# Adelaide-Autonomous-Racing-Kit/ac-mpc

Hardware: AMD Instinct MI355X
Metric: candidate-trajectories/sec (horizon=50) (higher is better)
Workload: dtype f32; 1 GPU; monza (synthetic circuit): 4096 candidates x horizon 50 per solve per GPU, 4096 solves (poses) batched per launch (256 distinct poses); mode S rollout + cost + argmin + winner record; horizon=50, mode=S, layout=U[P][n][2][N], parallelism=candidate-sharded x1, one all-reduce(MIN) of 4096 packed keys per step

## Files before the change

### ac-mpc_amd/acmpc_amd/_capi.py

```python
from __future__ import annotations

import ctypes as C
import os
import threading
from typing import Optional

import numpy as np

from . import _build

OK, EINVAL, EHIP, ENODEVICE, ECAPACITY, ESTATE = 0, -1, -2, -3, -4, -5
MODE_SPATIAL, MODE_TEMPORAL, MODE_DYNAMIC = 0, 1, 2
DYNAMICS_COUNT = 26
MAX_VEHICLES = 8
MAX_SUBSTEPS = 16
MAX_LOG_STEPS = 512
MAX_GRIP_HYPOTHESES = 65536
ENSEMBLE_MEAN, ENSEMBLE_MAX = 0, 1
ENSEMBLE_REDUCE = {"mean": ENSEMBLE_MEAN, "max": ENSEMBLE_MAX}
LAYOUT_CANDIDATE_MAJOR, LAYOUT_STEP_MAJOR = 0, 1
COEF_STRIDE = {MODE_SPATIAL: 12, MODE_TEMPORAL: 8, MODE_DYNAMIC: 8}
STATE_FLOATS = {MODE_SPATIAL: 3, MODE_TEMPORAL: 3, MODE_DYNAMIC: 6}
REC_COST, REC_VIOLATION, REC_NFEASIBLE, REC_OWNER, REC_HEADER = 0, 1, 2, 3, 4
ROUND_SINGLE, ROUND_PAIR, ROUND_QUAD, ROUND_TRIO = 0, 1, 2, 3
ROUND_FIELDS = ("kernel", "fused_finalize", "traced", "chained", "frames_in_lds", "frames_tabulated", "tick_accepted",
                "tick_frames")


ROLLOUT_KERNELS = (("step", None), ("tile", None), ("rows", "lds"), ("rows", "scalar"))


class EngineError(RuntimeError):

    def __init__(self, code: int, message: str):
        super().__init__("acmpc error %d: %s" % (code, message))
        self.code = code


class Params(C.Structure):
    _fields_ = [
        ("struct_size", C.c_uint32),
        ("mode", C.c_int32),
        ("device", C.c_int32),
        ("max_problems", C.c_int32),
        ("max_candidates", C.c_int32),
        ("max_steps", C.c_int32),
        ("nn_back", C.c_int32),
        ("nn_ahead", C.c_int32),
        ("centre_update", C.c_int32),
        ("lq_candidate", C.c_int32),
        ("step_cost", C.c_double * 3),
        ("r_term", C.c_double * 2),
        ("final_cost", C.c_double * 3),
        ("u_min", C.c_double * 2),
        ("u_max", C.c_double * 2),
        ("margin", C.c_double),
        ("wheelbase", C.c_double),
# ... 969 lines not shown
```

### ac-mpc_amd/csrc/acmpc_capi.hip

```cpp
#include <cstdio>
#include <cstdlib>
#include <algorithm>
#include <new>

#include "acmpc_ctx.h"
#include "acmpc_frames.h"
#include "acmpc_lq.h"

using namespace acmpc::capi;

namespace {

thread_local std::string g_create_error;

}

namespace acmpc {
namespace capi __attribute__((visibility("hidden"))) {

int fail(const acmpc_ctx* ctx, int code, const std::string& msg) {
  if (ctx != nullptr) {
    ctx->err = msg;
  } else {
    g_create_error = msg;
// ... 213 lines not shown
  c->touched_device = true;
  const acmpc_params& p = c->prm;
  const size_t cand = static_cast<size_t>(p.max_problems) * p.max_candidates;
  ACMPC_HIP(c, alloc_once(&c->d_centre, static_cast<size_t>(p.max_problems) * p.max_steps * 2 * sizeof(float)));
  ACMPC_HIP(c, alloc_once(&c->d_uref, static_cast<size_t>(p.max_problems) * p.max_steps * 2 * sizeof(float)));
  if (c->stream == nullptr) ACMPC_HIP(c, hipStreamCreateWithFlags(&c->stream, hipStreamNonBlocking));
  if (p.mode != ACMPC_MODE_DYNAMIC) {
    ACMPC_TRY(ensure_matrix(c));
  }
  const size_t state_floats = p.mode == ACMPC_MODE_DYNAMIC ? acmpc::kDynamicStateFloats : 3;
  ACMPC_HIP(c, alloc_once(&c->d_x0, static_cast<size_t>(p.max_problems) * state_floats * sizeof(float)));
  ACMPC_HIP(c, alloc_once(&c->d_costs, cand * sizeof(float)));
  ACMPC_HIP(c, alloc_once(&c->d_records,
                          static_cast<size_t>(p.max_problems) * acmpc_record_floats(p.max_steps) * sizeof(float)));
  ACMPC_HIP(c, alloc_once(&c->d_keys, static_cast<size_t>(p.max_problems) * sizeof(int64_t)));
  ACMPC_TRY(ensure_tail_buffers(c));
  ACMPC_HIP(c, host_alloc_once(&c->h_keys, static_cast<size_t>(p.max_problems) * sizeof(int64_t)));
  ACMPC_HIP(c, host_alloc_once(&c->h_io, (static_cast<size_t>(p.max_problems) * (state_floats + acmpc_record_floats(p.max_steps)) + 4) * sizeof(float)));
  if (p.lq_candidate != 0 && c->h_lq == nullptr) {
    const size_t lq_bytes = static_cast<size_t>(p.max_problems) * p.max_steps * 2 * sizeof(float);
    ACMPC_HIP(c, host_alloc_once(&c->h_lq, lq_bytes));
    std::memset(c->h_lq, 0, lq_bytes);
  }
  c->staging_ready = true;
  return ACMPC_OK;
}

static const char* const kOptionNames[] = {
    "ACMPC_SHAPE", "ACMPC_T_PACK", "ACMPC_NO_TILE", "ACMPC_TILE_ROWS", "ACMPC_TILE_TABLE", "ACMPC_NO_TRIO_ROUNDS",
    "ACMPC_NO_QUAD_ROUNDS", "ACMPC_NO_PAIR_ROUNDS", "ACMPC_SOLO_REGISTERS", "ACMPC_SOLO_SPLIT", "ACMPC_NO_VERIFIED_SEARCH",
    "ACMPC_NO_SOLO", "ACMPC_NO_FUSED_FINALIZE", "ACMPC_NO_TRACED_FINALIZE", "ACMPC_NO_CHAINED_ROUNDS", "ACMPC_NO_GRAPH",
    "ACMPC_NO_FUSED_SAMPLING", "ACMPC_TICK_GRAPH", "ACMPC_TICK_NO_FLAG", "ACMPC_TICK_NO_INLINE_PATH", "ACMPC_NO_ZERO_COPY", "ACMPC_TAILED_ROLLOUT", "ACMPC_NO_GROUP_FINALIZE", "ACMPC_FINALIZE_WAVES",
    "ACMPC_NO_CHAINED_STREAM", "ACMPC_LQ_BOX_ITERATIONS", "ACMPC_START_CLOCKS", "ACMPC_DYNAMIC_MATRIX_ROUNDS",
    "ACMPC_CONFORMANT_SYNC"};

static bool apply_option(acmpc_ctx* c, const char* name, const char* value) {
  const std::string key(name);
  const bool present = value != nullptr && value[0] != '\0';
  const bool on = present && !(value[0] == '0' && value[1] == '\0');
  auto tri = [&](int* field) { *field = present ? (value[0] == '1' ? 1 : 0) : -1; return true; };
  acmpc::LaunchOptions& o = c->opt;
  if (key == "ACMPC_SHAPE") {
    o.shape_block = o.shape_cpt = 0;
    if (present && std::sscanf(value, "%d,%d", &o.shape_block, &o.shape_cpt) != 2) o.shape_block = o.shape_cpt = 0;
    return true;
  }
  if (key == "ACMPC_T_PACK") { o.temporal_pack = present ? (value[0] == '1' ? 1 : 2) : 0; return true; }
  if (key == "ACMPC_NO_TILE") { o.no_tile = on; return true; }
  if (key == "ACMPC_TILE_ROWS") { o.tile_rows = present ? std::atoi(value) : -1; return true; }
  if (key == "ACMPC_TILE_TABLE") { o.tile_table = present ? (value[0] == 'l' ? 1 : 2) : 0; return true; }
  if (key == "ACMPC_NO_TRIO_ROUNDS") { o.no_trio_rounds = on; return true; }
  if (key == "ACMPC_NO_QUAD_ROUNDS") { o.no_quad_rounds = on; return true; }
  if (key == "ACMPC_NO_PAIR_ROUNDS") { o.no_pair_rounds = on; return true; }
  if (key == "ACMPC_SOLO_REGISTERS") return tri(&o.solo_registers);
  if (key == "ACMPC_SOLO_SPLIT") return tri(&o.solo_split);
  if (key == "ACMPC_NO_GROUP_FINALIZE") { o.no_group_finalize = on; return true; }
  if (key == "ACMPC_FINALIZE_WAVES") { o.finalize_waves = on; return true; }
  acmpc_ctx::Switches& w = c->sw;
  if (key == "ACMPC_NO_VERIFIED_SEARCH") { w.no_verified_search = on; return true; }
  if (key == "ACMPC_NO_SOLO") { w.no_solo = on; return true; }
  if (key == "ACMPC_NO_FUSED_FINALIZE") { w.no_fused_finalize = on; return true; }
  if (key == "ACMPC_NO_TRACED_FINALIZE") { w.no_traced_finalize = on; return true; }
  if (key == "ACMPC_NO_CHAINED_ROUNDS") { w.no_chained_rounds = on; return true; }
  if (key == "ACMPC_NO_CHAINED_STREAM") { w.no_chained_stream = on; return true; }
  if (key == "ACMPC_NO_GRAPH") { w.no_graph = on; return true; }
  if (key == "ACMPC_NO_FUSED_SAMPLING") { w.no_fused_sampling = on; return true; }
  if (key == "ACMPC_TICK_GRAPH") { w.tick_graph = on; return true; }
  if (key == "ACMPC_TICK_NO_FLAG") { w.tick_no_flag = on; return true; }
  if (key == "ACMPC_TICK_NO_INLINE_PATH") { w.tick_no_inline_path = on; return true; }
  if (key == "ACMPC_NO_ZERO_COPY") { w.no_zero_copy = on; return true; }
  if (key == "ACMPC_TAILED_ROLLOUT") { w.tailed_rollout = on; return true; }
  if (key == "ACMPC_START_CLOCKS") { c->want_start_clocks = on; return true; }
  if (key == "ACMPC_DYNAMIC_MATRIX_ROUNDS") { w.dynamic_matrix_rounds = on; return true; }
  if (key == "ACMPC_CONFORMANT_SYNC") {
    w.no_solo = w.no_fused_finalize = w.no_chained_stream = w.tick_no_flag = on;
    if (on) w.tailed_rollout = false;
    return true;
  }
  if (key == "ACMPC_LQ_BOX_ITERATIONS") { c->lq_box_iterations = present ? std::max(0, std::atoi(value)) : 40; return true; }
  return false;
}

}
}

extern "C" {
// ... 319 lines not shown
```

### ac-mpc_amd/csrc/acmpc_capi_optimize.hip

```cpp
#include <algorithm>

#include "acmpc_ctx.h"
#include "acmpc_lq.h"

using namespace acmpc::capi;

namespace acmpc {
namespace capi __attribute__((visibility("hidden"))) {

static const float* own_frames(const acmpc_ctx* c) { return c->h_nn_frames.empty() ? nullptr : c->d_nn_frames; }

bool use_fused_finalize(const acmpc_ctx* c, int n) {
  return !c->sw.no_fused_finalize && acmpc::fused_finalize_fits(c->prm.mode, n);
}

RoundPlan plan_rounds(const acmpc_ctx* c, int P, int N, int n) {
  const int blocks = (N + 63) / 64;
  RoundPlan plan{};
  plan.fused_finalize = use_fused_finalize(c, n);
  plan.traced = plan.fused_finalize && !c->sw.no_traced_finalize && acmpc::traced_finalize_fits(c->prm.mode, n) &&
                static_cast<long long>(P) * blocks <= kTraceBlocks;
  plan.chained = plan.traced && blocks <= acmpc::kChainBlocks && !c->sw.no_chained_rounds;
  return plan;
}

bool lq_plan_into(acmpc_ctx* c, const double* table, int n, const double start[3], float* out, bool start_is_pose, int problem) {
  double x0[3] = {start[0], start[1], start[2]};
  if (start_is_pose || c->prm.mode == ACMPC_MODE_TEMPORAL) acmpc::lq::frenet_start(table, n, start, x0);
  const float lo[2] = {c->w.ulo0, c->w.ulo1}, hi[2] = {c->w.uhi0, c->w.uhi1};
  const bool finite_start = std::isfinite(x0[0]) && std::isfinite(x0[1]) && std::isfinite(x0[2]);
  if (finite_start && acmpc::lq::plan(table, n, x0, c->prm.step_cost, c->prm.r_term, c->prm.final_cost, lo, hi, out)) {
    if (c->prm.lq_candidate == 2) {
      if (c->lq_box_state.size() <= static_cast<size_t>(problem)) c->lq_box_state.resize(static_cast<size_t>(problem) + 1);
      c->lq_box_last = acmpc::lqbox::refine(table, n, x0, c->prm.step_cost, c->prm.r_term, c->prm.final_cost, lo, hi,
                                            c->prm.margin, c->prm.w_bound, c->lq_box_iterations,
                                            c->lq_box_state[static_cast<size_t>(problem)], c->lq_box_ws, out);
    }
    return true;
  }
  if (c->prm.lq_candidate == 2 && c->lq_box_state.size() > static_cast<size_t>(problem))
    c->lq_box_state[static_cast<size_t>(problem)].reset();
  const double *kappa = table + 3 * static_cast<size_t>(n), *vel = table + 6 * static_cast<size_t>(n);
  for (int i = 0; i < n; ++i) {
    out[2 * i] = std::fmin(std::fmax(static_cast<float>(vel[i]), lo[0]), hi[0]);
    out[2 * i + 1] = std::fmin(std::fmax(static_cast<float>(kappa[i]), lo[1]), hi[1]);
  }
  return false;
}

int enqueue_rounds(acmpc_ctx* c, const OptInputs& in, int P, int N, int n, int rounds, double sigma_v, double sigma_k,
                   double shrink, uint64_t seed, const uint32_t* d_seed, hipStream_t s, bool fused, float* final_records,
                   unsigned* done, unsigned done_value) {
  const bool has_uref = in.uref != nullptr;
// ... 75 lines not shown
  ACMPC_HIP(c, hipMemcpyAsync(c->d_centre, centre, path_bytes, hipMemcpyHostToDevice, s));
  if (u_ref != nullptr) ACMPC_HIP(c, hipMemcpyAsync(c->d_uref, u_ref, path_bytes, hipMemcpyHostToDevice, s));
  double scale = 1.0;
  for (int r = 0; r < rounds; ++r, scale *= shrink) {
    RoundCentre from;
    ACMPC_TRY(round_centre(c, r, u_ref != nullptr, P, n, s, &from));
    if (c->sw.dynamic_matrix_rounds) {
      ACMPC_TRY(matrix_round(c, c->d_x0, from, nullptr, nullptr, P, N, n, r, rounds, sigma[0] * scale, sigma[1] * scale, seed, s));
      continue;
    }
    ACMPC_TRY(rollout_sampled_dynamic(c, c->d_x0, from.centre, from.stride, from.ref, P, N, n, 0, sigma[0] * scale, sigma[1] * scale,
                                      seed, static_cast<uint32_t>(r), softmin ? c->d_costs : nullptr, s));
    const Regenerate regen{from.centre, from.stride, from.ref,
                           make_spec(c, sigma[0] * scale, sigma[1] * scale, seed, static_cast<uint32_t>(r))};
    ACMPC_TRY(finalize(c, nullptr, softmin ? c->d_keys : nullptr, c->d_x0, nullptr, P, N, n, layout, 0, c->d_records,
                       acmpc::dynamic_blocks_per_problem(P, N, c->vehicles.K), s, &regen));
    if (softmin && r + 1 < rounds) {
      ACMPC_TRY(softmin_sampled(c, c->d_costs, c->d_keys, from.centre, from.stride, from.ref, P, N, n, 0, sigma[0] * scale,
                                sigma[1] * scale, seed, static_cast<uint32_t>(r), c->d_centre, nullptr, s));
    }
  }
  ACMPC_HIP(c, hipMemcpyAsync(records, c->d_records, static_cast<size_t>(P) * rec_floats * sizeof(float),
                              hipMemcpyDeviceToHost, s));
  ACMPC_HIP(c, hipStreamSynchronize(s));
  return ACMPC_OK;
}

}
}

extern "C" {

static_assert(acmpc::kSampledSingle == ACMPC_ROUND_SINGLE && acmpc::kSampledPair == ACMPC_ROUND_PAIR &&
              acmpc::kSampledQuad == ACMPC_ROUND_QUAD && acmpc::kSampledTrio == ACMPC_ROUND_TRIO, "include/acmpc.h");

int acmpc_describe_rounds(const acmpc_ctx* c, int32_t P, int32_t N, int32_t n, int32_t out[8]) {
  if (c == nullptr) return ACMPC_EINVAL;
  if (out == nullptr) return fail(c, ACMPC_EINVAL, "null output");
  if (c->prm.mode == ACMPC_MODE_DYNAMIC) return fail(c, ACMPC_ESTATE, "mode D has no sampled rounds of these forms");
  if (P < 1 || N < 1 || n < 1) return fail(c, ACMPC_EINVAL, "P, N and n must be positive");
  if (P > c->prm.max_problems || N > c->prm.max_candidates || n > c->prm.max_steps)
    return fail(c, ACMPC_ECAPACITY, "shape exceeds the handle's capacity");
  const bool tabulated = paths_tabulate_frames(c, n);
  const bool fused = !c->sw.no_fused_sampling && c->prm.centre_update == 0;
  const RoundPlan plan = fused ? plan_rounds(c, P, N, n) : RoundPlan{};
  const acmpc::SampledForm form = acmpc::choose_sampled_form(c->prm.mode, n, plan.traced, plan.fused_finalize,
                                                             tabulated && !c->sw.no_verified_search, c->opt);
  const char* why = nullptr;
  out[0] = fused ? form.kernel : -1;
  out[1] = plan.fused_finalize ? 1 : 0;
  out[2] = plan.traced ? 1 : 0;
  out[3] = plan.chained ? 1 : 0;
  out[4] = (fused && form.frames) ? 1 : 0;
  out[5] = tabulated ? 1 : 0;
  out[6] = tick_check(c, n + 1, 1, N, &why) == ACMPC_OK ? 1 : 0;
  out[7] = (out[6] != 0 && tick_tabulates_frames(c, n)) ? 1 : 0;
  return ACMPC_OK;
}

int acmpc_optimize(acmpc_ctx* c, const float* x0, const float* centre, const float* u_ref, int32_t P, int32_t N,
                   int32_t n, int32_t rounds, const double sigma[2], double shrink, uint64_t seed, float* records) {
  if (c == nullptr) return ACMPC_EINVAL;
  if (x0 == nullptr || centre == nullptr || sigma == nullptr || records == nullptr)
    return fail(c, ACMPC_EINVAL, "null argument");
  if (rounds < 1) return fail(c, ACMPC_EINVAL, "rounds must be positive");
  const int layout = ACMPC_LAYOUT_STEP_MAJOR;
  ACMPC_TRY(check_shape(c, P, N, n, layout));
  if (c->prm.mode == ACMPC_MODE_DYNAMIC && c->prm.centre_update == 1 && !(c->prm.softmin_lambda > 0.0))
    return fail(c, ACMPC_EINVAL, "softmin_lambda must be positive");
  ACMPC_TRY(ensure_device(c));
  ACMPC_TRY(ensure_staging(c));
  if (c->prm.mode == ACMPC_MODE_DYNAMIC) {
    return optimize_dynamic(c, x0, centre, u_ref, P, N, n, rounds, sigma, shrink, seed, records);
  }
  hipStream_t s = c->stream;
  const size_t x0_bytes = static_cast<size_t>(P) * 3 * sizeof(float);
  const size_t path_bytes = static_cast<size_t>(P) * n * 2 * sizeof(float);
  const size_t table_bytes = static_cast<size_t>(P) * n * c->coef_stride * sizeof(float);
  const size_t rec_bytes = static_cast<size_t>(P) * acmpc_record_floats(n) * sizeof(float);
  const bool has_uref = u_ref != nullptr;
// ... 96 lines not shown
```

### ac-mpc_amd/csrc/acmpc_kernels.h

```cpp
#pragma once
#include <hip/hip_runtime.h>
#include <stdint.h>

#include "acmpc_device.h"

namespace acmpc {

struct RolloutArgs {
  const float* U;
  const float* x0;
  const float* coef;
  const float* nn_frames;
  float* costs;
  int64_t* partial_keys;
  int* partial_feas;
  int P, N, n;
  int64_t index_offset;
  Weights w;
  int even_progress = 0;
  unsigned long long* start_clock = nullptr;
};

struct FinalizeArgs {
  const float* U;
// ... 25 lines not shown
  float* mean;
  double* weight_sum;
  int chunks;
  int P, N, n;
  float lambda;
};

constexpr int kSampleKnots = kKnots;

struct SampleArgs {
  const float* centre;
  const float* u_ref;
  const float* u_extra;
  float* U;
  int centre_stride;
  int P, N, n;
  int64_t index_offset;
  SampleSpec spec;
  const int64_t* prev_keys;
  const float* prev_trace;
  int prev_blocks;
  int prev_pitch;
};
constexpr int kTileRowsMaxSteps = 80;
constexpr int kChainBlocks = 256;

struct LaunchOptions {
  int shape_block = 0, shape_cpt = 0;
  int temporal_pack = 0;
  bool no_tile = false;
  int tile_rows = -1;
  int tile_table = 0;
  bool no_trio_rounds = false, no_quad_rounds = false, no_pair_rounds = false;
  int solo_registers = -1, solo_split = -1;
  bool no_group_finalize = false;
  bool finalize_waves = false;
};

struct LaunchShape {
  int block;
  int cpt;
  int blocks_per_problem;
  bool tile;
  int tile_waves;
  int pack;
  int tile_table = 0;
};

LaunchShape choose_shape(int P, int N, int layout, int mode, int n, const LaunchOptions& opt = LaunchOptions());
int max_blocks_per_problem(int N);
size_t tile_lds_bytes(int mode, int n);

hipError_t launch_rollout(int mode, int layout, const LaunchShape& shape, const RolloutArgs& args, hipStream_t s,
                          hipEvent_t start = nullptr, hipEvent_t stop = nullptr);
hipError_t launch_rollout_temporal_plain(const LaunchShape& shape, const RolloutArgs& args, hipStream_t s,
                                         hipEvent_t start, hipEvent_t stop);
hipError_t launch_rollout_tile_rows_plain(const LaunchShape& shape, const RolloutArgs& args, hipStream_t s,
                                          hipEvent_t start, hipEvent_t stop);
bool tile_rows_table_in_lds(const LaunchShape& shape, int P, int n);
hipError_t launch_finalize(int mode, int layout, const FinalizeArgs& args, hipStream_t s,
                           const LaunchOptions& opt = LaunchOptions());
bool chained_rollout_fits(int mode, int layout, const LaunchShape& shape, int P, const FinalizeArgs& fin, int fin_layout);
hipError_t launch_rollout_chained(int layout, const LaunchShape& shape, const RolloutArgs& args, const FinalizeArgs& fin,
                                  int fin_layout, hipStream_t s, hipEvent_t e0, hipEvent_t e1);
bool tailed_rollout_fits(int mode, int layout, const LaunchShape& shape, int n);
hipError_t launch_rollout_tailed(int layout, const LaunchShape& shape, const RolloutArgs& args, const FinalizeArgs& fin,
                                 int* tickets, hipStream_t s, hipEvent_t start = nullptr, hipEvent_t stop = nullptr);
hipError_t launch_sample(int layout, const SampleArgs& args, hipStream_t s);
constexpr int kTicketGroups = 8;
constexpr int kTicketStride = 64;
constexpr int kTicketGroupsMax = 32;
constexpr int kSoloBlocks = 1024;
struct FusedFinalize {
  int* tickets;
  float* records;
  bool controls_only;
  float* trace;
  int trace_pitch;
  unsigned* done;
  unsigned done_value;
  int64_t* keys_out = nullptr;
  int ticket_groups = 0;
};

enum SampledKernel { kSampledSingle = 0, kSampledPair = 1, kSampledQuad = 2, kSampledTrio = 3 };
struct SampledForm {
  int kernel;
  bool frames;
  size_t lds;
  int offset[3];
};
SampledForm choose_sampled_form(int mode, int n, bool traced, bool tail, bool frames, const LaunchOptions& opt = LaunchOptions());
hipError_t launch_rollout_sampled(int mode, const RolloutArgs& rollout, const SampleArgs& sample,
                                  const FusedFinalize& fused, hipStream_t s, hipEvent_t start = nullptr,
                                  hipEvent_t stop = nullptr, const LaunchOptions& opt = LaunchOptions());
bool solo_fits(int P, int N, int n, int layout, const LaunchOptions& opt = LaunchOptions());
int solo_trace_floats(int n);
hipError_t launch_rollout_solo(int layout, const RolloutArgs& args, const FusedFinalize& fused, hipStream_t s,
                               hipEvent_t start = nullptr, hipEvent_t stop = nullptr,
                               const LaunchOptions& opt = LaunchOptions());
int trace_floats(int n);
bool trio_frames_fit(int n);
bool traced_finalize_fits(int mode, int n);
bool fused_finalize_fits(int mode, int n);
int softmin_chunks(int N);
hipError_t launch_softmin(int layout, const SoftminArgs& args, hipStream_t s);
hipError_t launch_softmin_sampled(const SoftminArgs& args, const SampleArgs& sample, hipStream_t s);

}
```

### ac-mpc_amd/csrc/acmpc_kernels.hip

```cpp
#include "acmpc_rollout.h"

namespace acmpc {

namespace {

template <int LAYOUT>
__global__ void __launch_bounds__(256) sample_kernel(const SampleArgs a) {
  const int p = blockIdx.y;
  const int c = blockIdx.x * 256 + threadIdx.x;
  const int n = a.n;
  const SampleSpec sp = a.spec;
  const uint32_t gidx = static_cast<uint32_t>(a.index_offset + c);
  float z[kKnots][2];
  draw_normals(sp, gidx, static_cast<uint32_t>(p), z);
  const float* alt = (gidx == 1u) ? a.u_ref : (gidx == 2u) ? a.u_extra : nullptr;
  const bool use_ref = alt != nullptr;
  const float amp = use_ref ? 0.0f : candidate_amplitude(gidx);
  const float* __restrict__ centre =
      use_ref ? alt + static_cast<size_t>(p) * n * 2 : a.centre + static_cast<size_t>(p) * a.centre_stride;
  extern __shared__ __attribute__((aligned(16))) float s_smp[];
  float* s_w0 = s_smp;
  float* s_centre = s_smp + ((n + 3) & ~3);
  for (int e = threadIdx.x; e < n; e += 256) s_w0[e] = sp.segments[2 * e + 1];
  const float* __restrict__ block_centre = a.centre + static_cast<size_t>(p) * a.centre_stride;
// ... 1518 lines not shown
        }
        temporal_cost(st, s_wp + j * kCoefT, col[(2 * i) * kWave], col[(2 * i + 1) * kWave], w);
      }
    }
    if (t <= chunks) __syncthreads();
  }
  const float cost = finish_temporal<float>(st, n, w);
  s_trace[(5 * n) * kWave + lane] = st.V;
  s_trace[(5 * n + 1) * kWave + lane] = cost;
  if (active && a.costs != nullptr) a.costs[static_cast<size_t>(p) * a.N + c] = cost;
  const int64_t own_key = active ? pack_key(cost, static_cast<uint32_t>(a.index_offset + c)) : kKeyMax;
  int best_lane;
  const int64_t key = wave_min_key_by_lane(own_key, best_lane);
  const int nfeas = wave_sum_int((active && st.V == 0.0f) ? 1 : 0);
  {
    __syncthreads();
    float* trace_out = fused.trace + (static_cast<size_t>(p) * gridDim.x + blockIdx.x) * fused.trace_pitch;
    const float ox = coef[0], oy = coef[1];
    for (int e = lane; e < 5 * n + 2; e += kWave) {
      const int k = e - 2 * n;
      const bool is_x = k >= 0 && k < 3 * n && k % 3 == 0, is_y = k >= 0 && k < 3 * n && k % 3 == 1;
      const float value = s_trace[e * kWave + best_lane];
      publish(&trace_out[e], is_x ? value + ox : is_y ? value + oy : value);
    }
  }
  if (lane == 0) {
    const size_t slot = static_cast<size_t>(p) * gridDim.x + blockIdx.x;
    publish(&a.partial_keys[slot], key);
    publish(&a.partial_feas[slot], nfeas);
  }
  fused_tail<1>(a, smp, fused, true, nullptr);
}

}

bool tailed_rollout_fits(int mode, int layout, const LaunchShape& shape, int n) {
  const size_t rec_floats = static_cast<size_t>(4 + 2 * n + 3 * (n + 1));
  return mode == 0 && layout == 1 && !shape.tile && shape.block == 256 && (shape.cpt == 1 || shape.cpt == 2 || shape.cpt == 4) &&
         64 + rec_floats * sizeof(float) <= 64 * 1024;
}

hipError_t launch_rollout_tailed(int layout, const LaunchShape& shape, const RolloutArgs& args, const FinalizeArgs& fin,
                                 int* tickets, hipStream_t s, hipEvent_t e0, hipEvent_t e1) {
  clear_stale_error();
  if (!tailed_rollout_fits(0, layout, shape, args.n) || tickets == nullptr) return hipErrorInvalidValue;
  const dim3 grid(shape.blocks_per_problem, args.P);
  const size_t lds = 64 + static_cast<size_t>(4 + 2 * args.n + 3 * (args.n + 1)) * sizeof(float);
  if (shape.cpt == 1) return launch_kernel(rollout_tailed_kernel<0, 1, 1, 256, 1>, grid, dim3(256), lds, s, e0, e1, args, fin, tickets);
  if (shape.cpt == 2) return launch_kernel(rollout_tailed_kernel<0, 1, 2, 256, 2>, grid, dim3(256), lds, s, e0, e1, args, fin, tickets);
  return launch_kernel(rollout_tailed_kernel<0, 1, 4, 256, 2>, grid, dim3(256), lds, s, e0, e1, args, fin, tickets);
}

bool chained_rollout_fits(int mode, int layout, const LaunchShape& shape, int P, const FinalizeArgs& fin, int fin_layout) {
  const int fin_groups = (fin.P + kFinalizeWaves - 1) / kFinalizeWaves;
  const int rows = (fin_groups + std::max(shape.blocks_per_problem, 1) - 1) / std::max(shape.blocks_per_problem, 1);
  return rows <= P && static_cast<long long>(P) + rows <= 65535 && mode == 0 && layout == 1 && !shape.tile && shape.block == 256 && (shape.cpt == 1 || shape.cpt == 2 || shape.cpt == 4) &&
         !fin.controls_only && fin.records != nullptr && fin.keys_in == nullptr && fin.P >= 1 && (fin.regenerate || fin_layout == 1) &&
         kFinalizeWaves * group_finalize_floats(fin.n, 1) * sizeof(float) <= 20 * 1024;
}

hipError_t launch_rollout_chained(int layout, const LaunchShape& shape, const RolloutArgs& args, const FinalizeArgs& fin,
                                  int fin_layout, hipStream_t s, hipEvent_t e0, hipEvent_t e1) {
  clear_stale_error();
  if (!chained_rollout_fits(0, layout, shape, args.P, fin, fin_layout)) return hipErrorInvalidValue;
  const int groups = (fin.P + kFinalizeWaves - 1) / kFinalizeWaves;
  const int fin_rows = (groups + shape.blocks_per_problem - 1) / shape.blocks_per_problem;
// ... 34 lines not shown
  clear_stale_error();
  const dim3 grid((args.N + 255) / 256, args.P);
  const size_t sample_lds = (((static_cast<size_t>(args.n) + 3) & ~static_cast<size_t>(3)) + 2 * args.n) * sizeof(float);
  if (layout == 0) return launch_kernel(sample_kernel<0>, grid, dim3(256), sample_lds, s, nullptr, nullptr, args);
  if (layout == 1) return launch_kernel(sample_kernel<1>, grid, dim3(256), sample_lds, s, nullptr, nullptr, args);
  return hipErrorInvalidValue;
}

namespace {
size_t sampled_rollout_floats(int mode, int n) {
  return (mode == 1) ? ((static_cast<size_t>(n) * (kCoefT + kKeyStride) + 3) & ~static_cast<size_t>(3)) : 0;
}
size_t sampled_uniform_floats(int mode, int n) {
  return static_cast<size_t>(n) * ((mode == 0 ? kCoefS : 0) + 7) + 4;
}
size_t sampled_finalize_floats(int mode, int n) {
  const size_t rec_floats = static_cast<size_t>(4 + 2 * n + 3 * (n + 1));
  return ((rec_floats + 3) & ~static_cast<size_t>(3)) + (mode == 1 ? static_cast<size_t>(n) * (kCoefT + kKeyStride) : 0);
}
}

bool fused_finalize_fits(int mode, int n) {
  return (sampled_rollout_floats(mode, n) + sampled_finalize_floats(mode, n) + sampled_uniform_floats(mode, n)) *
             sizeof(float) <= 64 * 1024;
}

int trace_floats(int n) { return 5 * n + 2; }

bool traced_finalize_fits(int mode, int n) {
  return (sampled_rollout_floats(mode, n) + static_cast<size_t>(trace_floats(n)) * kWave +
          sampled_uniform_floats(mode, n)) * sizeof(float) <= 160 * 1024;
}

SampledForm choose_sampled_form(int mode, int n, bool traced, bool tail, bool frames, const LaunchOptions& opt) {
  constexpr size_t kBudget = 160u * 1024u;
  SampledForm form{};
  const size_t rollout_floats = sampled_rollout_floats(mode, n);
  const size_t trace = static_cast<size_t>(trace_floats(n)) * kWave;
  const size_t finalize_floats = traced ? trace : tail ? sampled_finalize_floats(mode, n) : 0;
  const size_t uniform_floats = sampled_uniform_floats(mode, n);
  form.kernel = kSampledSingle;
  form.lds = (rollout_floats + finalize_floats + uniform_floats) * sizeof(float);
  form.offset[0] = static_cast<int>(rollout_floats);
  form.offset[1] = static_cast<int>(rollout_floats + finalize_floats);
  if (form.lds > kBudget) return form;
  if (mode == 1 && traced && !opt.no_trio_rounds) {
    const size_t plain_tables = (static_cast<size_t>(n) * (kCoefT + kKeyStride) + 3) & ~static_cast<size_t>(3);
    const size_t uniform = (static_cast<size_t>(n) * 7 + 4 + 3) & ~static_cast<size_t>(3);
    const size_t index = (static_cast<size_t>(n) * kWave / 2 + 3) & ~static_cast<size_t>(3);
    bool with_frames = frames && n >= kVerifiedWindow;
    size_t tables = plain_tables + (with_frames ? static_cast<size_t>(verified_frame_floats(n)) : 0);
    if ((tables + trace + uniform + index) * sizeof(float) > kBudget) {
      with_frames = false;
      tables = plain_tables;
    }
    const size_t trio_lds = (tables + trace + uniform + index) * sizeof(float);
    if (trio_lds <= kBudget) {
      form.kernel = kSampledTrio;
      form.frames = with_frames;
      form.lds = trio_lds;
      form.offset[0] = static_cast<int>(tables);
      form.offset[1] = static_cast<int>(tables + trace);
      form.offset[2] = static_cast<int>(tables + trace + uniform);
      return form;
    }
  }
  if (mode == 0 && traced && !opt.no_quad_rounds && !opt.no_pair_rounds) {
    const size_t uniform = (uniform_floats + 3) & ~static_cast<size_t>(3);
    const size_t quad_lds = (trace + uniform + static_cast<size_t>(2 * kKnots + 1) * kWave) * sizeof(float);
    if (quad_lds <= kBudget) {
      form.kernel = kSampledQuad;
      form.lds = quad_lds;
      form.offset[0] = static_cast<int>(trace);
      form.offset[1] = static_cast<int>(trace + uniform);
      return form;
    }
  }
  if (mode == 0 && traced && !opt.no_pair_rounds) {
    const size_t exchange = static_cast<size_t>(2) * kPairChunk * kPairValues * kWave;
    const size_t pair_lds = (trace + uniform_floats + exchange) * sizeof(float);
    if (pair_lds <= kBudget) {
      form.kernel = kSampledPair;
      form.lds = pair_lds;
      form.offset[0] = static_cast<int>(trace);
      form.offset[1] = static_cast<int>(trace + uniform_floats);
      return form;
    }
  }
  return form;
}

bool trio_frames_fit(int n) { return choose_sampled_form(1, n, true, true, true, LaunchOptions()).frames; }

hipError_t launch_rollout_sampled(int mode, const RolloutArgs& rollout, const SampleArgs& sample,
                                  const FusedFinalize& fused, hipStream_t s, hipEvent_t e0, hipEvent_t e1,
                                  const LaunchOptions& opt) {
  clear_stale_error();
  const int n = rollout.n;
  const dim3 grid((rollout.N + kWave - 1) / kWave, rollout.P);
  const bool traced = fused.trace != nullptr;
  if (mode != 0 && mode != 1) return hipErrorInvalidValue;
  const SampledForm form = choose_sampled_form(mode, n, traced, fused.tickets != nullptr, rollout.nn_frames != nullptr, opt);
  if (form.lds > 160u * 1024u) return hipErrorInvalidValue;
  if (traced && fused.trace_pitch < trace_floats(n)) return hipErrorInvalidValue;
  if (form.kernel == kSampledTrio) {
    RolloutArgs rollout_trio = rollout;
    if (!form.frames) rollout_trio.nn_frames = nullptr;
    return launch_kernel_lds<&rollout_sampled_trio_kernel>(grid, dim3(3 * kWave), form.lds, s, e0, e1, rollout_trio, sample,
                                                           fused, form.offset[0], form.offset[1], form.offset[2]);
  }
  if (form.kernel == kSampledQuad)
    return launch_kernel_lds<&rollout_sampled_quad_kernel>(grid, dim3(kQuadWaves * kWave), form.lds, s, e0, e1, rollout,
                                                           sample, fused, form.offset[0], form.offset[1]);
  if (form.kernel == kSampledPair)
    return launch_kernel_lds<&rollout_sampled_pair_kernel>(grid, dim3(2 * kWave), form.lds, s, e0, e1, rollout, sample,
                                                           fused, form.offset[0], form.offset[1]);
  if (mode == 0)
    return launch_kernel_lds<&rollout_sampled_kernel<0>>(grid, dim3(kWave), form.lds, s, e0, e1, rollout, sample, fused,
                                                         form.offset[0], form.offset[1]);
  return launch_kernel_lds<&rollout_sampled_kernel<1>>(grid, dim3(kWave), form.lds, s, e0, e1, rollout, sample, fused,
                                                       form.offset[0], form.offset[1]);
}

}
```

### include/acmpc.h

```cpp
#ifndef ACMPC_H
#define ACMPC_H

#include <stdint.h>

#ifdef __cplusplus
extern "C" {
#endif

#define ACMPC_OK 0
#define ACMPC_EINVAL (-1)
#define ACMPC_EHIP (-2)
#define ACMPC_ENODEVICE (-3)
#define ACMPC_ECAPACITY (-4)
#define ACMPC_ESTATE (-5)

#define ACMPC_MODE_SPATIAL 0
#define ACMPC_MODE_TEMPORAL 1
#define ACMPC_MODE_DYNAMIC 2

#define ACMPC_LAYOUT_CANDIDATE_MAJOR 0
#define ACMPC_LAYOUT_STEP_MAJOR 1

#define ACMPC_COEF_STRIDE_SPATIAL 12
#define ACMPC_COEF_STRIDE_TEMPORAL 8
// ... 160 lines not shown
  int32_t qp_check_every;
  int32_t qp_method;
  double offset;
  double v_min, v_max, a_min, a_max, ay_max, ki_min, end_velocity;
  double sigma[2];
  double shrink;
  double qp_eps_abs, qp_eps_rel;
  uint64_t seed;
  int32_t map_index;
  int32_t centreline_points;
  double pose_x, pose_y;
  double lateral_offset;
} acmpc_tick;

int acmpc_bind_map(acmpc_ctx* ctx, const double* centre, int32_t M, double spacing);
int acmpc_map_reference_path(acmpc_ctx* ctx, int32_t map_index, double pose_x, double pose_y, double lateral_offset,
                             int32_t horizon, int32_t centreline_points, double* coords, int32_t* first_index);

int acmpc_control_tick(acmpc_ctx* ctx, const acmpc_tick* tick, const double* coords, const float* centre, double* table,
                       float* record, double* decision, double* projected_control, double* prediction,
                       double* cum_time, double* times, double* accelerations, double* steer_rates, double* info,
                       double* coords_out);

int acmpc_tick_read_device_tables(acmpc_ctx* ctx, float* x0, float* u_ref, float* coef);
int acmpc_tick_read_device_frames(acmpc_ctx* ctx, float* out, int64_t capacity_floats);
int acmpc_speed_profile_qp_device(acmpc_ctx* ctx, const double* v_hi, const double* ds, int32_t n, double a_min,
                                  double a_max, double v_min, int32_t max_iter, int32_t check_every, double eps_abs,
                                  double eps_rel, double* v, double* y, int32_t warm_start, int32_t* iterations);

#define ACMPC_ROUND_SINGLE 0
#define ACMPC_ROUND_PAIR 1
#define ACMPC_ROUND_QUAD 2
#define ACMPC_ROUND_TRIO 3
int acmpc_describe_rounds(const acmpc_ctx* ctx, int32_t P, int32_t N, int32_t n, int32_t out[8]);

#define ACMPC_ROLLOUT_STEP 0
#define ACMPC_ROLLOUT_TILE 1
#define ACMPC_ROLLOUT_ROWS_LDS 2
#define ACMPC_ROLLOUT_ROWS_SCALAR 3
int acmpc_describe_rollout(const acmpc_ctx* ctx, int32_t P, int32_t N, int32_t n, int32_t layout, int32_t out[8]);

int acmpc_waypoint_table(const double* coords, int32_t H, double eps, double* table);
int acmpc_velocity_ceiling(const double* kappa, int32_t n, double ay_max, double ki_min, double v_min, double v_max,
                           int32_t localised, int32_t has_end_velocity, double end_velocity, double* ceiling);
int acmpc_unpack_decision(const double* z, int32_t n, const double* table, double wheelbase, double* projected_control,
                          double* prediction, double* cum_time, double* times, double* accelerations,
                          double* steer_rates);
int acmpc_unpack_decision_temporal(const double* z, int32_t n, double dt, double wheelbase, double* projected_control,
                                   double* prediction, double* cum_time, double* times, double* accelerations,
                                   double* steer_rates);

int32_t acmpc_search_window(int32_t* back);
int32_t acmpc_search_frame_floats(int32_t n);
int acmpc_search_frames(const float* coef, int32_t P, int32_t n, float* out, int64_t capacity_floats);

void acmpc_philox4x32(const uint32_t counter[4], const uint32_t key[2], uint32_t out[4]);

int acmpc_speed_profile_qp(const double* v_hi, const double* ds, int32_t n, double a_min, double a_max, double v_min,
                           int32_t max_iter, int32_t check_every, double eps_abs, double eps_rel, double* v, double* y,
                           int32_t warm_start, int32_t* iterations);

int acmpc_speed_profile_exact(const double* v_hi, const double* ds, int32_t n, double a_min, double a_max, double v_min,
                              double* v, double* y);

int acmpc_rollout_start_clocks(acmpc_ctx* ctx, uint64_t* out, int32_t capacity, int32_t* count);

// ... 60 lines not shown
```

Measured before the change: 15.70 billion candidate-trajectories/s.

## Add many-workgroup batch sampled rollout kernel for large spatial candidate counts

Adds a new sampled rollout kernel for spatial mode. It uses 256-thread workgroups and two candidates per lane, packed as f32x2 arithmetic, and reduces min keys and feasible counts inside the workgroup before publishing per-block partials to the fused finalize tail. It is selected automatically when problems times candidates reaches 131072, and when selected it disables the traced and chained finalize paths. The goal is higher occupancy and more instruction-level parallelism for big batches, at the cost of losing the traced-finalize shortcut and writing more partial slots.

```diff
diff --git a/ac-mpc_amd/acmpc_amd/_capi.py b/ac-mpc_amd/acmpc_amd/_capi.py
--- a/ac-mpc_amd/acmpc_amd/_capi.py
+++ b/ac-mpc_amd/acmpc_amd/_capi.py
@@ -22,7 +22,7 @@
 COEF_STRIDE = {MODE_SPATIAL: 12, MODE_TEMPORAL: 8, MODE_DYNAMIC: 8}
 STATE_FLOATS = {MODE_SPATIAL: 3, MODE_TEMPORAL: 3, MODE_DYNAMIC: 6}
 REC_COST, REC_VIOLATION, REC_NFEASIBLE, REC_OWNER, REC_HEADER = 0, 1, 2, 3, 4
-ROUND_SINGLE, ROUND_PAIR, ROUND_QUAD, ROUND_TRIO = 0, 1, 2, 3
+ROUND_SINGLE, ROUND_PAIR, ROUND_QUAD, ROUND_TRIO, ROUND_BATCH = 0, 1, 2, 3, 4
 ROUND_FIELDS = ("kernel", "fused_finalize", "traced", "chained", "frames_in_lds", "frames_tabulated", "tick_accepted",
                 "tick_frames")
 
diff --git a/ac-mpc_amd/csrc/acmpc_capi.hip b/ac-mpc_amd/csrc/acmpc_capi.hip
--- a/ac-mpc_amd/csrc/acmpc_capi.hip
+++ b/ac-mpc_amd/csrc/acmpc_capi.hip
@@ -269,6 +269,7 @@
     "ACMPC_NO_SOLO", "ACMPC_NO_FUSED_FINALIZE", "ACMPC_NO_TRACED_FINALIZE", "ACMPC_NO_CHAINED_ROUNDS", "ACMPC_NO_GRAPH",
     "ACMPC_NO_FUSED_SAMPLING", "ACMPC_TICK_GRAPH", "ACMPC_TICK_NO_FLAG", "ACMPC_TICK_NO_INLINE_PATH", "ACMPC_NO_ZERO_COPY", "ACMPC_TAILED_ROLLOUT", "ACMPC_NO_GROUP_FINALIZE", "ACMPC_FINALIZE_WAVES",
     "ACMPC_NO_CHAINED_STREAM", "ACMPC_LQ_BOX_ITERATIONS", "ACMPC_START_CLOCKS", "ACMPC_DYNAMIC_MATRIX_ROUNDS",
+    "ACMPC_NO_BATCH_ROUNDS", "ACMPC_BATCH_ROUNDS",
     "ACMPC_CONFORMANT_SYNC"};
 
 static bool apply_option(acmpc_ctx* c, const char* name, const char* value) {
@@ -289,6 +290,8 @@
   if (key == "ACMPC_NO_TRIO_ROUNDS") { o.no_trio_rounds = on; return true; }
   if (key == "ACMPC_NO_QUAD_ROUNDS") { o.no_quad_rounds = on; return true; }
   if (key == "ACMPC_NO_PAIR_ROUNDS") { o.no_pair_rounds = on; return true; }
+  if (key == "ACMPC_NO_BATCH_ROUNDS") { o.no_batch_rounds = on; return true; }
+  if (key == "ACMPC_BATCH_ROUNDS") { o.batch_rounds = on; return true; }
   if (key == "ACMPC_SOLO_REGISTERS") return tri(&o.solo_registers);
   if (key == "ACMPC_SOLO_SPLIT") return tri(&o.solo_split);
   if (key == "ACMPC_NO_GROUP_FINALIZE") { o.no_group_finalize = on; return true; }
diff --git a/ac-mpc_amd/csrc/acmpc_capi_optimize.hip b/ac-mpc_amd/csrc/acmpc_capi_optimize.hip
--- a/ac-mpc_amd/csrc/acmpc_capi_optimize.hip
+++ b/ac-mpc_amd/csrc/acmpc_capi_optimize.hip
@@ -18,7 +18,8 @@
   const int blocks = (N + 63) / 64;
   RoundPlan plan{};
   plan.fused_finalize = use_fused_finalize(c, n);
-  plan.traced = plan.fused_finalize && !c->sw.no_traced_finalize && acmpc::traced_finalize_fits(c->prm.mode, n) &&
+  const bool batch = plan.fused_finalize && acmpc::batch_round_applies(c->prm.mode, static_cast<long long>(P) * N, c->opt);
+  plan.traced = plan.fused_finalize && !batch && !c->sw.no_traced_finalize && acmpc::traced_finalize_fits(c->prm.mode, n) &&
                 static_cast<long long>(P) * blocks <= kTraceBlocks;
   plan.chained = plan.traced && blocks <= acmpc::kChainBlocks && !c->sw.no_chained_rounds;
   return plan;
@@ -160,7 +161,9 @@
 extern "C" {
 
 static_assert(acmpc::kSampledSingle == ACMPC_ROUND_SINGLE && acmpc::kSampledPair == ACMPC_ROUND_PAIR &&
-              acmpc::kSampledQuad == ACMPC_ROUND_QUAD && acmpc::kSampledTrio == ACMPC_ROUND_TRIO, "include/acmpc.h");
+              acmpc::kSampledQuad == ACMPC_ROUND_QUAD && acmpc::kSampledTrio == ACMPC_ROUND_TRIO &&
+              acmpc::kSampledBatch == ACMPC_ROUND_BATCH, "include/acmpc.h");
+static_assert(acmpc::kBatchCandidates > 64LL * kTraceBlocks, "no launch of the many-workgroup form's size leaves traces");
 
 int acmpc_describe_rounds(const acmpc_ctx* c, int32_t P, int32_t N, int32_t n, int32_t out[8]) {
   if (c == nullptr) return ACMPC_EINVAL;
@@ -173,7 +176,8 @@
   const bool fused = !c->sw.no_fused_sampling && c->prm.centre_update == 0;
   const RoundPlan plan = fused ? plan_rounds(c, P, N, n) : RoundPlan{};
   const acmpc::SampledForm form = acmpc::choose_sampled_form(c->prm.mode, n, plan.traced, plan.fused_finalize,
-                                                             tabulated && !c->sw.no_verified_search, c->opt);
+                                                             tabulated && !c->sw.no_verified_search, c->opt,
+                                                             static_cast<long long>(P) * N);
   const char* why = nullptr;
   out[0] = fused ? form.kernel : -1;
   out[1] = plan.fused_finalize ? 1 : 0;
diff --git a/ac-mpc_amd/csrc/acmpc_kernels.h b/ac-mpc_amd/csrc/acmpc_kernels.h
--- a/ac-mpc_amd/csrc/acmpc_kernels.h
+++ b/ac-mpc_amd/csrc/acmpc_kernels.h
@@ -81,6 +81,8 @@
   int tile_rows = -1;
   int tile_table = 0;
   bool no_trio_rounds = false, no_quad_rounds = false, no_pair_rounds = false;
+  bool no_batch_rounds = false;
+  bool batch_rounds = false;
   int solo_registers = -1, solo_split = -1;
   bool no_group_finalize = false;
   bool finalize_waves = false;
@@ -132,14 +134,18 @@
   int ticket_groups = 0;
 };
 
-enum SampledKernel { kSampledSingle = 0, kSampledPair = 1, kSampledQuad = 2, kSampledTrio = 3 };
+enum SampledKernel { kSampledSingle = 0, kSampledPair = 1, kSampledQuad = 2, kSampledTrio = 3, kSampledBatch = 4 };
 struct SampledForm {
   int kernel;
   bool frames;
   size_t lds;
   int offset[3];
 };
-SampledForm choose_sampled_form(int mode, int n, bool traced, bool tail, bool frames, const LaunchOptions& opt = LaunchOptions());
+SampledForm choose_sampled_form(int mode, int n, bool traced, bool tail, bool frames, const LaunchOptions& opt = LaunchOptions(),
+                                long long candidates = 0);
+constexpr long long kBatchCandidates = 131072;
+bool batch_round_applies(int mode, long long candidates, const LaunchOptions& opt);
+int batch_blocks_per_problem(int N);
 hipError_t launch_rollout_sampled(int mode, const RolloutArgs& rollout, const SampleArgs& sample,
                                   const FusedFinalize& fused, hipStream_t s, hipEvent_t start = nullptr,
                                   hipEvent_t stop = nullptr, const LaunchOptions& opt = LaunchOptions());
diff --git a/ac-mpc_amd/csrc/acmpc_kernels.hip b/ac-mpc_amd/csrc/acmpc_kernels.hip
--- a/ac-mpc_amd/csrc/acmpc_kernels.hip
+++ b/ac-mpc_amd/csrc/acmpc_kernels.hip
@@ -1574,6 +1574,128 @@
   fused_tail<1>(a, smp, fused, true, nullptr);
 }
 
+#ifndef ACMPC_BATCH_CPT
+#define ACMPC_BATCH_CPT 2
+#endif
+#ifndef ACMPC_BATCH_WAVES
+#define ACMPC_BATCH_WAVES 6
+#endif
+constexpr int kBatchBlock = 256;
+constexpr int kBatchCpt = ACMPC_BATCH_CPT;
+
+template <int CPT, bool SPECIAL>
+__device__ __forceinline__ void roll_drawn(const RolloutArgs& a, const SampleArgs& smp, const int p, const uint32_t g0,
+                                           float (&cost)[CPT], float (&viol)[CPT]) {
+  using F = typename std::conditional<CPT == 2, f32x2, float>::type;
+  static_assert(CPT == 1 || CPT == 2, "one arithmetic state per lane");
+  const int n = a.n;
+  const Weights w = a.w;
+  const SampleSpec sp = smp.spec;
+  const float* __restrict__ coef = a.coef + static_cast<size_t>(p) * n * kCoefS;
+  const float* __restrict__ x0 = a.x0 + p * 3;
+  const float* __restrict__ centre = smp.centre + static_cast<size_t>(p) * smp.centre_stride;
+  const float* __restrict__ knot_weight = sp.segments;
+  float z[CPT][kKnots][2];
+  float amp[CPT];
+  const float* own[CPT];
+#pragma unroll
+  for (int j = 0; j < CPT; ++j) {
+    const uint32_t gidx = g0 + static_cast<uint32_t>(j);
+    draw_normals(sp, gidx, static_cast<uint32_t>(p), z[j]);
+    const bool use_extra = (gidx == 2u) && (smp.u_extra != nullptr);
+    const bool use_ref = (gidx == 1u) && (smp.u_ref != nullptr);
+    amp[j] = (use_ref || use_extra) ? 0.0f : candidate_amplitude(gidx);
+    own[j] = use_extra ? smp.u_extra + static_cast<size_t>(p) * n * 2
+             : use_ref ? smp.u_ref + static_cast<size_t>(p) * n * 2
+                       : centre;
+  }
+  StateS_<F> st{splat<F>(x0[0]), splat<F>(x0[1]), splat<F>(x0[2]), splat<F>(0.0f), splat<F>(0.0f)};
+#pragma unroll
+  for (int knot = 0; knot < kKnots - 1; ++knot) {
+#pragma unroll 2
+    for (int i = sp.knot_begin[knot]; i < sp.knot_begin[knot + 1]; ++i) {
+      const float* __restrict__ row = coef + i * kCoefS;
+      const float w0 = knot_weight[2 * i + 1];
+      float v[CPT], k[CPT];
+#pragma unroll
+      for (int j = 0; j < CPT; ++j) {
+        const float cv = SPECIAL ? own[j][2 * i] : centre[2 * i];
+        const float ck = SPECIAL ? own[j][2 * i + 1] : centre[2 * i + 1];
+        blend_control(sp, amp[j], w0, cv, ck, z[j][knot][0], z[j][knot][1], z[j][knot + 1][0], z[j][knot + 1][1], v[j], k[j]);
+      }
+      if constexpr (CPT == 2) {
+        F vv, kk;
+        vv[0] = v[0], vv[1] = v[1], kk[0] = k[0], kk[1] = k[1];
+        step_spatial<F>(st, row, vv, kk, w);
+      } else {
+        step_spatial<F>(st, row, v[0], k[0], w);
+      }
+    }
+  }
+  const F total = finish_spatial<F>(st, w);
+  if constexpr (CPT == 2) {
+    cost[0] = total[0], cost[1] = total[1], viol[0] = st.V[0], viol[1] = st.V[1];
+  } else {
+    cost[0] = total, viol[0] = st.V;
+  }
+}
+
+template <int CPT>
+__global__ void __launch_bounds__(kBatchBlock, ACMPC_BATCH_WAVES) rollout_sampled_batch_kernel(const RolloutArgs a, const SampleArgs smp,
+                                                                                              const FusedFinalize fused) {
+  extern __shared__ __attribute__((aligned(16))) unsigned char s_batch[];
+  int64_t* s_key = reinterpret_cast<int64_t*>(s_batch);
+  int* s_feas = reinterpret_cast<int*>(s_batch + 32);
+  const int p = blockIdx.y;
+  const int tid = threadIdx.x;
+  const int c0 = (static_cast<int>(blockIdx.x) * kBatchBlock + tid) * CPT;
+  float cost[CPT], viol[CPT];
+#pragma unroll
+  for (int j = 0; j < CPT; ++j) {
+    cost[j] = __builtin_inff();
+    viol[j] = 1.0f;
+  }
+  if (c0 < a.N) {
+    const uint32_t first = static_cast<uint32_t>(a.index_offset + static_cast<int64_t>(blockIdx.x) * (kBatchBlock * CPT));
+    const bool special = (smp.u_ref != nullptr || smp.u_extra != nullptr) && (first <= 2u || first > 0u - static_cast<uint32_t>(kBatchBlock * CPT));
+    const uint32_t g0 = static_cast<uint32_t>(a.index_offset + c0);
+    if (special) roll_drawn<CPT, true>(a, smp, p, g0, cost, viol);
+    else roll_drawn<CPT, false>(a, smp, p, g0, cost, viol);
+  }
+  int64_t key = kKeyMax;
+  int nfeas = 0;
+#pragma unroll
+  for (int j = 0; j < CPT; ++j) {
+    if (c0 + j < a.N) {
+      if (a.costs != nullptr) a.costs[static_cast<size_t>(p) * a.N + c0 + j] = cost[j];
+      const int64_t kj = pack_key(cost[j], static_cast<uint32_t>(a.index_offset + c0 + j));
+      key = (kj < key) ? kj : key;
+      nfeas += (viol[j] == 0.0f) ? 1 : 0;
+    }
+  }
+  key = wave_min_key(key);
+  nfeas = wave_sum_int(nfeas);
+  const int lane = tid & (kWave - 1);
+  const int wave = tid / kWave;
+  if (lane == 0) {
+    s_key[wave] = key;
+    s_feas[wave] = nfeas;
+  }
+  __syncthreads();
+  if (tid >= kWave) return;
+  if (tid == 0) {
+#pragma unroll
+    for (int q = 1; q < kBatchBlock / kWave; ++q) {
+      key = (s_key[q] < key) ? s_key[q] : key;
+      nfeas += s_feas[q];
+    }
+    const size_t slot = static_cast<size_t>(p) * gridDim.x + blockIdx.x;
+    publish(&a.partial_keys[slot], key);
+    publish(&a.partial_feas[slot], nfeas);
+  }
+  fused_tail<0>(a, smp, fused, false, reinterpret_cast<float*>(s_batch + 64));
+}
+
 }
 
 bool tailed_rollout_fits(int mode, int layout, const LaunchShape& shape, int n) {
@@ -1674,9 +1796,21 @@
           sampled_uniform_floats(mode, n)) * sizeof(float) <= 160 * 1024;
 }
 
-SampledForm choose_sampled_form(int mode, int n, bool traced, bool tail, bool frames, const LaunchOptions& opt) {
+bool batch_round_applies(int mode, long long candidates, const LaunchOptions& opt) {
+  return mode == 0 && !opt.no_batch_rounds && (opt.batch_rounds || candidates >= kBatchCandidates);
+}
+
+int batch_blocks_per_problem(int N) { return (N + kBatchBlock * kBatchCpt - 1) / (kBatchBlock * kBatchCpt); }
+
+SampledForm choose_sampled_form(int mode, int n, bool traced, bool tail, bool frames, const LaunchOptions& opt,
+                                long long candidates) {
   constexpr size_t kBudget = 160u * 1024u;
   SampledForm form{};
+  if (!traced && tail && batch_round_applies(mode, candidates, opt)) {
+    form.kernel = kSampledBatch;
+    form.lds = 64 + sampled_finalize_floats(mode, n) * sizeof(float);
+    return form;
+  }
   const size_t rollout_floats = sampled_rollout_floats(mode, n);
   const size_t trace = static_cast<size_t>(trace_floats(n)) * kWave;
   const size_t finalize_floats = traced ? trace : tail ? sampled_finalize_floats(mode, n) : 0;
@@ -1742,9 +1876,16 @@
   const dim3 grid((rollout.N + kWave - 1) / kWave, rollout.P);
   const bool traced = fused.trace != nullptr;
   if (mode != 0 && mode != 1) return hipErrorInvalidValue;
-  const SampledForm form = choose_sampled_form(mode, n, traced, fused.tickets != nullptr, rollout.nn_frames != nullptr, opt);
+  const SampledForm form = choose_sampled_form(mode, n, traced, fused.tickets != nullptr, rollout.nn_frames != nullptr, opt,
+                                               static_cast<long long>(rollout.P) * rollout.N);
   if (form.lds > 160u * 1024u) return hipErrorInvalidValue;
   if (traced && fused.trace_pitch < trace_floats(n)) return hipErrorInvalidValue;
+  if (form.kernel == kSampledBatch) {
+    if (sample.prev_keys != nullptr) return hipErrorInvalidValue;
+    const dim3 batch_grid(batch_blocks_per_problem(rollout.N), rollout.P);
+    return launch_kernel(rollout_sampled_batch_kernel<kBatchCpt>, batch_grid, dim3(kBatchBlock), form.lds, s, e0, e1, rollout,
+                         sample, fused);
+  }
   if (form.kernel == kSampledTrio) {
     RolloutArgs rollout_trio = rollout;
     if (!form.frames) rollout_trio.nn_frames = nullptr;
diff --git a/include/acmpc.h b/include/acmpc.h
--- a/include/acmpc.h
+++ b/include/acmpc.h
@@ -216,6 +216,7 @@
 #define ACMPC_ROUND_PAIR 1
 #define ACMPC_ROUND_QUAD 2
 #define ACMPC_ROUND_TRIO 3
+#define ACMPC_ROUND_BATCH 4
 int acmpc_describe_rounds(const acmpc_ctx* ctx, int32_t P, int32_t N, int32_t n, int32_t out[8]);
 
 #define ACMPC_ROLLOUT_STEP 0
```

Result: no change. 15.89 billion candidate-trajectories/s (median of 4 runs) (+1.2%).
